# fal-ai-community/video-diffusion-speedrun

Hardware: AMD Instinct MI355X
Metric: train-step samples/sec (video latents) (higher is better)
Workload: dtype bf16; 1 GPU; C3b DiT-XL/2 bf16, latents [16,16,64,64] pt=2 -> 8192+16 tokens, ctx [512,4096]; per_gpu_batch=12, global_batch=12, parallelism=single, launch=eager, deterministic=False

## Files before the change

### video_diffusion_speedrun_amd/csrc/gemm.hip

```cpp
#include "common.h"
#include "prof.h"
#include "config.h"
#include "../../include/vds.h"
#include <cmath>
#include <cstdint>
#include <cstring>
#include <mutex>
#include <type_traits>

#ifndef VDS_GEMM_AUX_NT
#define VDS_GEMM_AUX_NT 1
#endif
namespace {

constexpr int BM = 128, BN = 128, BK = 64;
constexpr int TILE_BYTES = 16384;
constexpr int EPI_LD = 68;
constexpr int LDS_BYTES = 4 * 64 * EPI_LD * 4;
constexpr int GROUP_M = 8;

struct GemmP {
  int M, N, K;
  const bf16_t* A; long lda;
  const bf16_t* B; long ldb;
// ... 233 lines not shown
      const float g[8] = {g0[0], g0[1], g0[2], g0[3], g1[0], g1[1], g1[2], g1[3]};
      const u32x4 xr = auxr[it];
      u32x4 o, o2;
#pragma unroll
      for (int e = 0; e < 4; ++e) {
        float a = v[2 * e] + bias8[2 * e], bb = v[2 * e + 1] + bias8[2 * e + 1];
        o[e] = pack_bf2(a, bb);
        o2[e] = pack_bf2(bflo(xr[e]) + a * g[2 * e], bfhi(xr[e]) + bb * g[2 * e + 1]);
      }
      if (p.C) *reinterpret_cast<u32x4*>(reinterpret_cast<bf16_t*>(p.C) + grow * p.ldc + gcol) = o;
      *reinterpret_cast<u32x4*>(reinterpret_cast<bf16_t*>(p.C2) + grow * p.ldc2 + gcol) = o2;
    } else if constexpr (EPI == VDS_EPI_DGELU) {
      const u32x4 pr = auxr[it];
      u32x4 o;
#pragma unroll
      for (int e = 0; e < 4; ++e) {
        if constexpr (LUT) o[e] = f2_to_bf2(f32x2{v[2 * e], v[2 * e + 1]} * lut_pair(lut, pr[e]));
        else o[e] = pack_bf2(v[2 * e] * dgelu_f(bflo(pr[e])), v[2 * e + 1] * dgelu_f(bfhi(pr[e])));
      }
      if (p.C) *reinterpret_cast<u32x4*>(reinterpret_cast<bf16_t*>(p.C) + grow * p.ldc + gcol) = o;
      if constexpr (EMIT) ev = o;
    }
    if constexpr (EMIT) {
      float f[8];
#pragma unroll
      for (int e = 0; e < 4; ++e) { f[2 * e] = bflo(ev[e]); f[2 * e + 1] = bfhi(ev[e]); }
      if (p.e_colsum)
#pragma unroll
        for (int e = 0; e < 8; ++e) cs[e] += f[e];
      if (emit) {
#pragma unroll
        for (int e = 0; e < 8; ++e) {
          e_max = fmaxf(e_max, fabsf(f[e]));
          f[e] = fminf(fmaxf(f[e] * e_scale, -e_fmax), e_fmax);
        }
        const u32x2 w = {cvt4_fp8(p.e_fmt, f[0], f[1], f[2], f[3]), cvt4_fp8(p.e_fmt, f[4], f[5], f[6], f[7])};
        ew[it] = w;
        if (p.e_q) *reinterpret_cast<u32x2*>(p.e_q + grow * p.e_ldq + gcol) = w;
      }
    }
  }
  if constexpr (EMIT) {
    if (emit) {
      if (p.e_amax_out) {
#pragma unroll
        for (int o = 32; o > 0; o >>= 1) e_max = fmaxf(e_max, __shfl_xor(e_max, o));
        unsigned* a = reinterpret_cast<unsigned*>(p.e_amax_out);
        if (lane == 0 && __float_as_uint(e_max) > __atomic_load_n(a, __ATOMIC_RELAXED)) atomicMax(a, __float_as_uint(e_max));
      }
    }
  }
}

template <int EPI, int EFMT, bool C1, bool C2, bool EQ, bool CS, int WC = 64, int NIT = 8>
__device__ __forceinline__ void epilogue_full(const GemmP& p, const float* stg, const char* lut, int row0, int col0, int lane,
                                              float (&cs)[8], u32x2 (&ew)[NIT], const u32x4 (&auxr)[NIT], float e_scale,
                                              float& e_max) {
  const int c8 = lane & 7, rin = lane >> 3;
  if constexpr (WC < 64) {
    if (c8 * 8 >= WC) {
      if constexpr (EQ) {
#pragma unroll
        for (int it = 0; it < NIT; ++it) ew[it] = u32x2{0u, 0u};
      }
      return;
    }
  }
  const int gcol = col0 + c8 * 8;
  const long grow0 = row0 + rin;
  f32x2 bias[4];
#pragma unroll
  for (int e = 0; e < 4; ++e) bias[e] = f32x2{0.f, 0.f};
  if constexpr (EPI == VDS_EPI_STORE || EPI == VDS_EPI_BIAS_GELU || EPI == VDS_EPI_GATE_RES) {
    if (p.bias) {
      const u32x4 bv = *reinterpret_cast<const u32x4*>(p.bias + gcol);
#pragma unroll
      for (int e = 0; e < 4; ++e) bias[e] = bf2_to_f2(bv[e]);
    }
  }
  [[maybe_unused]] f32x2 g[4];
  if constexpr (EPI == VDS_EPI_GATE_RES) {
    const float* gp = p.gate + (long)((row0 + p.row_base) / p.rows_per_batch) * p.ldgate + gcol;
    const f32x4 g0 = *reinterpret_cast<const f32x4*>(gp), g1 = *reinterpret_cast<const f32x4*>(gp + 4);
    g[0] = f32x2{g0[0], g0[1]}; g[1] = f32x2{g0[2], g0[3]}; g[2] = f32x2{g1[0], g1[1]}; g[3] = f32x2{g1[2], g1[3]};
  }
  [[maybe_unused]] bf16_t* c1 = reinterpret_cast<bf16_t*>(p.C) + grow0 * p.ldc + gcol;
  [[maybe_unused]] bf16_t* c2 = reinterpret_cast<bf16_t*>(p.C2) + grow0 * p.ldc2 + gcol;
  [[maybe_unused]] unsigned char* eq = p.e_q + grow0 * p.e_ldq + gcol;
  const long s1 = 8 * p.ldc, s2 = 8 * p.ldc2, sq = 8 * p.e_ldq;
  constexpr float FMAX = EFMT == 0 ? 448.0f : 57344.0f;
  const float* sp = stg + rin * EPI_LD + c8 * 8;
#pragma unroll
  for (int it = 0; it < NIT; ++it) {
    const f32x4 lo = *reinterpret_cast<const f32x4*>(sp + it * 8 * EPI_LD);
    const f32x4 hi = *reinterpret_cast<const f32x4*>(sp + it * 8 * EPI_LD + 4);
    const f32x2 v[4] = {f32x2{lo[0], lo[1]}, f32x2{lo[2], lo[3]}, f32x2{hi[0], hi[1]}, f32x2{hi[2], hi[3]}};
    [[maybe_unused]] u32x4 ev;
    if constexpr (EPI == VDS_EPI_STORE) {
      u32x4 o;
#pragma unroll
      for (int e = 0; e < 4; ++e) o[e] = f2_to_bf2(v[e] + bias[e]);
      __builtin_nontemporal_store(o, reinterpret_cast<u32x4*>(c1 + it * s1));
    } else if constexpr (EPI == VDS_EPI_BIAS_GELU) {
      u32x4 o, o2;
#pragma unroll
      for (int e = 0; e < 4; ++e) {
        o[e] = f2_to_bf2(v[e] + bias[e]);
        o2[e] = f2_to_bf2(bf2_to_f2(o[e]) * lut_pair(lut, o[e]));
      }
      if constexpr (C1) __builtin_nontemporal_store(o, reinterpret_cast<u32x4*>(c1 + it * s1));
      if constexpr (C2) __builtin_nontemporal_store(o2, reinterpret_cast<u32x4*>(c2 + it * s2));
      ev = o2;
    } else if constexpr (EPI == VDS_EPI_GATE_RES) {
      const u32x4 xr = auxr[it];
      u32x4 o, o2;
#pragma unroll
      for (int e = 0; e < 4; ++e) {
        const f32x2 a = v[e] + bias[e];
        o[e] = f2_to_bf2(a);
        o2[e] = f2_to_bf2(bf2_to_f2(xr[e]) + a * g[e]);
      }
      if constexpr (C1) __builtin_nontemporal_store(o, reinterpret_cast<u32x4*>(c1 + it * s1));
      __builtin_nontemporal_store(o2, reinterpret_cast<u32x4*>(c2 + it * s2));
    } else if constexpr (EPI == VDS_EPI_DGELU) {
      const u32x4 pr = auxr[it];
      u32x4 o;
#pragma unroll
      for (int e = 0; e < 4; ++e) o[e] = f2_to_bf2(v[e] * lut_pair(lut, pr[e]));
      if constexpr (C1) __builtin_nontemporal_store(o, reinterpret_cast<u32x4*>(c1 + it * s1));
      ev = o;
    }
    if constexpr (EQ || CS) {
      f32x2 f[4];
#pragma unroll
      for (int e = 0; e < 4; ++e) f[e] = bf2_to_f2(ev[e]);
      if constexpr (CS)
#pragma unroll
        for (int e = 0; e < 4; ++e) { cs[2 * e] += f[e][0]; cs[2 * e + 1] += f[e][1]; }
      if constexpr (EQ) {
        float q[8];
#pragma unroll
        for (int e = 0; e < 4; ++e) {
          e_max = fmaxf(fmaxf(e_max, fabsf(f[e][0])), fabsf(f[e][1]));
          const f32x2 sc = f[e] * e_scale;
          q[2 * e] = __builtin_amdgcn_fmed3f(sc[0], -FMAX, FMAX);
          q[2 * e + 1] = __builtin_amdgcn_fmed3f(sc[1], -FMAX, FMAX);
        }
        const u32x2 w = {fp8_cvt4<EFMT>(q[0], q[1], q[2], q[3]), fp8_cvt4<EFMT>(q[4], q[5], q[6], q[7])};
        ew[it] = w;
        *reinterpret_cast<u32x2*>(eq + it * sq) = w;
      }
    }
  }
}

template <int EPI, bool EMIT, int WC = 64, int NIT = 8>
__device__ __forceinline__ bool epilogue_full_dispatch(const GemmP& p, const float* stg, const char* lut, int row0, int col0,
                                                       int lane, float (&cs)[8], u32x2 (&ew)[NIT], const u32x4 (&auxr)[NIT],
                                                       float e_scale, float& e_max) {
  const bool c1 = p.C != nullptr, c2 = p.C2 != nullptr;
  [[maybe_unused]] bool eq = false, eany = false, csum = false;
  if constexpr (EMIT) {
    eq = p.e_q != nullptr;
    eany = p.e_q || p.e_qt;
    csum = p.e_colsum != nullptr;
  }
#define VDS_FULL(E, F, A, B, Q, S) epilogue_full<E, F, A, B, Q, S, WC, NIT>(p, stg, lut, row0, col0, lane, cs, ew, auxr, e_scale, e_max)
  if constexpr (EPI == VDS_EPI_STORE) {
    VDS_FULL(EPI, 0, true, false, false, false);
    return true;
  } else if constexpr (EPI == VDS_EPI_GATE_RES) {
    if (c1) VDS_FULL(EPI, 0, true, true, false, false);
    else VDS_FULL(EPI, 0, false, true, false, false);
    return true;
  } else if constexpr (EPI == VDS_EPI_BIAS_GELU) {
    if (c1 && c2 && !eany) { VDS_FULL(EPI, 0, true, true, false, false); return true; }
    if (!c1 && c2 && !eany) { VDS_FULL(EPI, 0, false, true, false, false); return true; }
    if constexpr (EMIT) {
      if (c1 && !c2 && eq && !csum && p.e_fmt == 0) { VDS_FULL(EPI, 0, true, false, true, false); return true; }
    }
    return false;
  } else if constexpr (EPI == VDS_EPI_DGELU) {
    if (c1 && !eany && !csum) { VDS_FULL(EPI, 0, true, false, false, false); return true; }
    if constexpr (EMIT) {
      if (c1 && !eany && csum) { VDS_FULL(EPI, 0, true, false, false, true); return true; }
      if (!c1 && eq && csum && p.e_fmt == 1) { VDS_FULL(EPI, 1, false, false, true, true); return true; }
      if (!c1 && eq && !csum && p.e_fmt == 1) { VDS_FULL(EPI, 1, false, false, true, false); return true; }
    }
    return false;
  } else {
    return false;
  }
#undef VDS_FULL
}

template <int LAYOUT, int EPI>
__global__ __launch_bounds__(256, 2) void gemm_kernel(GemmP p) {
  extern __shared__ __attribute__((aligned(16))) char smem[];
  constexpr bool A_KM = (LAYOUT == VDS_TN);
  constexpr bool B_KM = (LAYOUT != VDS_NT);
  const int tid = threadIdx.x, lane = tid & 63;
  const int wave = __builtin_amdgcn_readfirstlane(tid >> 6);
  const int wm = wave >> 1, wn = wave & 1;

  const int nwg = p.tiles_m * p.tiles_n;
  int pid = blockIdx.x;
  {
    int q = nwg >> 3, r = nwg & 7, xcd = pid & 7, idx = pid >> 3;
    pid = (xcd < r ? xcd * (q + 1) : r * (q + 1) + (xcd - r) * q) + idx;
  }
  const int group = GROUP_M * p.tiles_n;
  const int first_m = (pid / group) * GROUP_M;
  const int gsz = min(p.tiles_m - first_m, GROUP_M);
  const int tile_m = first_m + (pid % group) % gsz;
  const int tile_n = (pid % group) / gsz;
  const int m0 = tile_m * BM, n0 = tile_n * BN;

  const int kt_total = (p.K + BK - 1) / BK;
  int kt_begin = 0, kt_end = kt_total;
  if (p.split_k > 1) {
    int per = (kt_total + p.split_k - 1) / p.split_k;
    kt_begin = blockIdx.y * per;
    kt_end = min(kt_total, kt_begin + per);
    if (kt_begin >= kt_end) return;
  }

  const srd_t ra = make_srd(p.A, p.a_bytes);
  const srd_t rb = make_srd(p.B, p.b_bytes);
  unsigned va[4], vb[4];
  stage_offsets<A_KM>(va, wave, lane, p.lda, m0);
  stage_offsets<B_KM>(vb, wave, lane, p.ldb, n0);
  const unsigned a_step = A_KM ? (unsigned)(BK * p.lda * 2) : BK * 2;
  const unsigned b_step = B_KM ? (unsigned)(BK * p.ldb * 2) : BK * 2;


  f32x4 acc[4][4];
#pragma unroll
  for (int i = 0; i < 4; ++i)
#pragma unroll
    for (int j = 0; j < 4; ++j) acc[i][j] = f32x4{0.f, 0.f, 0.f, 0.f};

  stage_tile<A_KM>(ra, smem, va, kt_begin * a_step, wave, lane, p.K - kt_begin * BK);
  stage_tile<B_KM>(rb, smem + TILE_BYTES, vb, kt_begin * b_step, wave, lane, p.K - kt_begin * BK);
  VDS_WAIT_VM(0);
// ... 64 lines not shown

template <int G, int STRIDE, int OFF>
__device__ __forceinline__ int to_tile(int local) { return (local / G) * STRIDE + OFF + (local % G); }

__device__ __forceinline__ int swz8(int row) { return ((row >> 1) & 3) | ((row >> 3) & 4); }
__device__ __forceinline__ i32x8 frag_km8(const char* tile, int db, int lane) {
  const int m = lane & 15, g = lane >> 4, q = m >> 1, pp = m & 1;
  const int st = ((q >> 1) & 3) | ((g & 1) << 2);
  const char* p = tile + (32 * g + q) * 128 + ((db ^ st) << 4) + 8 * pp;
  i32x8 r;
#pragma unroll
  for (int t = 0; t < 4; ++t) {
    typedef __attribute__((ext_vector_type(2))) int i32x2_t;
    const i32x2_t w = __builtin_amdgcn_ds_read_tr8_b64_v2i32((__attribute__((address_space(3))) i32x2_t*)LDS_PTR(p + t * 8 * 128));
    r[2 * t] = w[0];
    r[2 * t + 1] = w[1];
  }
  return r;
}
template <int G, int STRIDE, int OFF>
__device__ __forceinline__ void half_offsets_km8(unsigned (&voff)[2], int (&kchunk)[2], int wave, int lane, long ld_bytes,
                                                 int origin) {
#pragma unroll
  for (int j = 0; j < 2; ++j) {
    const int row = (wave * 2 + j) * 8 + (lane >> 3);
    const int chunk = (lane & 7) ^ swz8(row);
    kchunk[j] = 0;
    voff[j] = (unsigned)((long)row * ld_bytes + origin + to_tile<G, STRIDE, OFF>(chunk * 16));
  }
}

template <bool KMAJOR, int G, int STRIDE, int OFF, int NP>
__device__ __forceinline__ void half_offsets(unsigned (&voff)[NP], int (&kchunk)[NP], int wave, int lane, long ld,
                                             int origin) {
#pragma unroll
  for (int j = 0; j < NP; ++j) {
    const int q = wave * NP + j;
    if constexpr (!KMAJOR) {
      const int row = q * 8 + (lane >> 3);
      const int chunk = swz_kc(row, lane & 7);
      kchunk[j] = chunk * 8;
      voff[j] = (unsigned)(((long)(origin + to_tile<G, STRIDE, OFF>(row)) * ld + chunk * 8) * 2);
    } else {
      static_assert(NP == 2, "half-tiles are staged as two 1-KiB pieces per wave");
      const int krow = q * 4 + (lane >> 4);
      const int pc = lane & 15;
      const int chunk = (((pc >> 1) ^ swz_km(krow)) << 1) | (pc & 1);
      kchunk[j] = 0;
      voff[j] = (unsigned)(((long)krow * ld + origin + to_tile<G, STRIDE, OFF>(chunk * 8)) * 2);
    }
  }
}

template <bool KMAJOR, int NP = 2>
__device__ __forceinline__ void issue_half(srd_t rsrc, char* slot, const unsigned (&voff)[NP],
                                           const int (&kchunk)[NP], unsigned koff, int krem, int wave) {
  const unsigned base = lds_addr_of(slot) + wave * (NP * 1024);
#pragma unroll
  for (int j = 0; j < NP; ++j) {
    unsigned off = voff[j] + koff;
    if constexpr (!KMAJOR) {
      if (kchunk[j] >= krem) off = 0xfffffff0u;
    } else {
      if (krem <= 0) off = 0xfffffff0u;
    }
    lds_dma16(rsrc, base + j * 1024, off);
  }
}

template <int LAYOUT, int EPI, int FMT, int WN>
__device__ __forceinline__ void gemm_tile(const GemmP& p, char* smem, const int m0, const int n0, const int kt_begin,
                                          const int kt_end) {
  static_assert(FMT == 0 || (FMT != 3 && LAYOUT == VDS_NT) || (FMT == 3 && LAYOUT == VDS_TN),
                "fp8 operands: k-contiguous (FMT 1 / 2, NT) or both k-major (FMT 3, TN: the weight gradient)");
  using G = Geo<WN>;
  constexpr int WCOLS = G::WCOLS, NJ = G::NJ, BUF = G::BUF;
  constexpr int SLOT_A0 = G::A0, SLOT_A1 = G::A1, SLOT_B0 = G::B0, SLOT_B1 = G::B1;
  constexpr int NPB1 = 2;
  constexpr bool A_KM = (LAYOUT == VDS_TN);
  constexpr bool B_KM = (LAYOUT != VDS_NT);
  const int tid = threadIdx.x, lane = tid & 63;
  const int wave = __builtin_amdgcn_readfirstlane(tid >> 6);
  const int wr = wave >> 2, wc = wave & 3;
  const srd_t ra = make_srd(p.A, p.a_bytes);
  const srd_t rb = make_srd(p.B, p.b_bytes);
  constexpr bool USE_LUT = EPI == VDS_EPI_BIAS_GELU || EPI == VDS_EPI_DGELU;
  char* const ring = smem + (USE_LUT ? LUT_BYTES : 0);
  if (USE_LUT) {
    const srd_t rl = make_srd(g_gelu_lut[EPI == VDS_EPI_DGELU ? 1 : 0], LUT_BYTES);
    const unsigned lb = lds_addr_of(smem) + wave * 2048;
    lds_dma16(rl, lb, (unsigned)(wave * 2048 + lane * 16));
    lds_dma16(rl, lb + 1024, (unsigned)(wave * 2048 + 1024 + lane * 16));
  }
  unsigned va[2][2], vb0[2], vb1[NPB1];
  int ca[2][2], cb0[2], cb1[NPB1];
  if constexpr (FMT == 3) {
    half_offsets_km8<64, 128, 0>(va[0], ca[0], wave, lane, 2 * p.lda, m0);
    half_offsets_km8<64, 128, 64>(va[1], ca[1], wave, lane, 2 * p.lda, m0);
    if constexpr (WN == 128) {
      half_offsets_km8<32, 32, 0>(vb0, cb0, wave, lane, 2 * p.ldb, n0);
    } else {
      half_offsets_km8<32, 64, 0>(vb0, cb0, wave, lane, 2 * p.ldb, n0);
      half_offsets_km8<32, 64, 32>(vb1, cb1, wave, lane, 2 * p.ldb, n0);
    }
  } else {
  half_offsets<A_KM, 64, 128, 0, 2>(va[0], ca[0], wave, lane, p.lda, m0);
  half_offsets<A_KM, 64, 128, 64, 2>(va[1], ca[1], wave, lane, p.lda, m0);
  }
  if constexpr (FMT == 3) {
  } else if constexpr (WN == 128) {
    half_offsets<B_KM, 32, 32, 0, 2>(vb0, cb0, wave, lane, p.ldb, n0);
  } else {
    half_offsets<B_KM, 32, 64, 0, 2>(vb0, cb0, wave, lane, p.ldb, n0);
    half_offsets<B_KM, 32, 64, 32, 2>(vb1, cb1, wave, lane, p.ldb, n0);
  }
  const unsigned a_step = A_KM ? (unsigned)((FMT == 3 ? 2 * BK : BK) * p.lda * 2) : BK * 2;
  const unsigned b_step = B_KM ? (unsigned)((FMT == 3 ? 2 * BK : BK) * p.ldb * 2) : BK * 2;

  auto issue = [&](int T, int which, int par) {
    const int krem = (T < kt_end) ? p.K - T * BK : 0;
    char* buf = ring + par * BUF;
    if (which == 0) issue_half<A_KM>(ra, buf + SLOT_A0, va[0], ca[0], (unsigned)T * a_step, krem, wave);
    else if (which == 3) issue_half<A_KM>(ra, buf + SLOT_A1, va[1], ca[1], (unsigned)T * a_step, krem, wave);
    else if (which == 1) issue_half<B_KM>(rb, buf + SLOT_B0, vb0, cb0, (unsigned)T * b_step, krem, wave);
    else if constexpr (WN != 128) issue_half<B_KM, NPB1>(rb, buf + SLOT_B1, vb1, cb1, (unsigned)T * b_step, krem, wave);
  };

  f32x4 acc[8][NJ];
#pragma unroll
  for (int i = 0; i < 8; ++i)
#pragma unroll
    for (int j = 0; j < NJ; ++j) {
      acc[i][j] = f32x4{0.f, 0.f, 0.f, 0.f};
      if constexpr (LAYOUT != VDS_TN) asm volatile("" : "+v"(acc[i][j]));
    }

  constexpr int KS = FMT == 0 ? 2 : 1;
  using frag_t = std::conditional_t<FMT == 0, bf16x8, i32x8>;
  auto mma = [&](const frag_t& a, const frag_t& b, f32x4 c) {
    if constexpr (FMT == 0) return __builtin_amdgcn_mfma_f32_16x16x32_bf16(b, a, c, 0, 0, 0);
    else return __builtin_amdgcn_mfma_scale_f32_16x16x128_f8f6f4(b, a, c, 0, FMT >= 2 ? 1 : 0, 0, 0, 0, 0);
  };
  auto read_a4 = [&](const char* slot, frag_t (&fa)[4][KS]) {
#pragma unroll
    for (int i = 0; i < 4; ++i)
#pragma unroll
      for (int ks = 0; ks < KS; ++ks) {
        if constexpr (FMT == 3) fa[i][ks] = frag_km8(slot, wr * 4 + i, lane);
        else if constexpr (FMT != 0) fa[i][ks] = frag_kc8(slot, wr * 64 + i * 16, lane);
        else if constexpr (A_KM) fa[i][ks] = frag_km(slot, wr * 64 + i * 16, ks, lane);
        else fa[i][ks] = frag_kc(slot, wr * 64 + i * 16, ks, lane);
      }
  };
  auto read_b2 = [&](const char* slot, frag_t (&fb)[2][KS]) {
#pragma unroll
    for (int j = 0; j < 2; ++j)
#pragma unroll
      for (int ks = 0; ks < KS; ++ks) {
        if constexpr (FMT == 3) fb[j][ks] = frag_km8(slot, wc * 2 + j, lane);
        else if constexpr (FMT != 0) fb[j][ks] = frag_kc8(slot, wc * 32 + j * 16, lane);
        else if constexpr (B_KM) fb[j][ks] = frag_km(slot, wc * 32 + j * 16, ks, lane);
        else fb[j][ks] = frag_kc(slot, wc * 32 + j * 16, ks, lane);
      }
  };

  if constexpr (WN == 256) {
  issue(kt_begin, 0, 0); issue(kt_begin, 1, 0); issue(kt_begin, 2, 0); issue(kt_begin, 3, 0);
  issue(kt_begin + 1, 0, 1); issue(kt_begin + 1, 1, 1); issue(kt_begin + 1, 2, 1);
  VDS_WAIT_VM(8);
  __builtin_amdgcn_s_barrier();
  if (wr == 1) __builtin_amdgcn_s_barrier();
  frag_t fa[4][KS], fb0[2][KS], fb1[2][KS];
  auto quad = [&](int qa, int qb, frag_t (&fb)[2][KS]) {
#pragma unroll
    for (int ks = 0; ks < KS; ++ks)
#pragma unroll
      for (int i = 0; i < 4; ++i)
#pragma unroll
        for (int j = 0; j < 2; ++j) acc[qa * 4 + i][qb * 2 + j] = mma(fa[i][ks], fb[j][ks], acc[qa * 4 + i][qb * 2 + j]);
  };
  auto k_tile = [&](int T, auto PAR) {
    constexpr int par = decltype(PAR)::value;
    const char* buf = ring + par * BUF;
    read_a4(buf + SLOT_A0, fa);
    read_b2(buf + SLOT_B0, fb0);
    read_b2(buf + SLOT_B1, fb1);
    issue(T + 1, 3, par ^ 1);
    VDS_WAIT_LGKM0();
    VDS_WAIT_VM(8);
    __builtin_amdgcn_s_barrier();
    __builtin_amdgcn_s_setprio(1);
    quad(0, 0, fb0);
    quad(0, 1, fb1);
    __builtin_amdgcn_s_setprio(0);
    __builtin_amdgcn_s_barrier();
    read_a4(buf + SLOT_A1, fa);
    issue(T + 2, 0, par);
    issue(T + 2, 1, par);
    issue(T + 2, 2, par);
    VDS_WAIT_LGKM0();
    VDS_WAIT_VM(8);
    __builtin_amdgcn_s_barrier();
    __builtin_amdgcn_s_setprio(1);
    quad(1, 1, fb1);
    quad(1, 0, fb0);
    __builtin_amdgcn_s_setprio(0);
    __builtin_amdgcn_s_barrier();
  };
  for (int T = kt_begin; T < kt_end; T += 2) {
    k_tile(T, std::integral_constant<int, 0>{});
    if (T + 1 < kt_end) k_tile(T + 1, std::integral_constant<int, 1>{});
  }
  } else {
  static_assert(WN == 128, "tile widths: 256, and 128 for a narrow last tile column");
  issue(kt_begin, 0, 0); issue(kt_begin, 1, 0); issue(kt_begin, 3, 0);
  issue(kt_begin + 1, 0, 1); issue(kt_begin + 1, 1, 1);
  VDS_WAIT_VM(6);
  __builtin_amdgcn_s_barrier();
  if (wr == 1) __builtin_amdgcn_s_barrier();
  frag_t fa[4][KS], fb0[2][KS];
  auto quad = [&](int qa) {
#pragma unroll
    for (int ks = 0; ks < KS; ++ks)
#pragma unroll
      for (int i = 0; i < 4; ++i)
#pragma unroll
        for (int j = 0; j < 2; ++j) acc[qa * 4 + i][j] = mma(fa[i][ks], fb0[j][ks], acc[qa * 4 + i][j]);
  };
  auto k_tile = [&](int T, auto PAR) {
    constexpr int par = decltype(PAR)::value;
    const char* buf = ring + par * BUF;
    read_a4(buf + SLOT_A0, fa);
    read_b2(buf + SLOT_B0, fb0);
    issue(T + 1, 3, par ^ 1);
    VDS_WAIT_LGKM0();
    VDS_WAIT_VM(6);
    __builtin_amdgcn_s_barrier();
    __builtin_amdgcn_s_setprio(1);
    quad(0);
    __builtin_amdgcn_s_setprio(0);
    __builtin_amdgcn_s_barrier();
    read_a4(buf + SLOT_A1, fa);
    issue(T + 2, 0, par);
    issue(T + 2, 1, par);
    VDS_WAIT_LGKM0();
    VDS_WAIT_VM(6);
    __builtin_amdgcn_s_barrier();
    __builtin_amdgcn_s_setprio(1);
    quad(1);
    __builtin_amdgcn_s_setprio(0);
    __builtin_amdgcn_s_barrier();
  };
  for (int T = kt_begin; T < kt_end; T += 2) {
    k_tile(T, std::integral_constant<int, 0>{});
    if (T + 1 < kt_end) k_tile(T + 1, std::integral_constant<int, 1>{});
  }
  }
  constexpr int NIT = 8;
  constexpr int NSTEP = 16 / NIT;
  constexpr int RSTEP = 8 * NIT;
  u32x4 auxr2[NSTEP][NIT];
#pragma unroll
  for (int st = 0; st < NSTEP; ++st)
    epilogue_prefetch<EPI, G::WCOLS, NIT>(p, m0 + wr * 128 + st * RSTEP, n0 + wc * G::WCOLS, lane, auxr2[st]);
  if (wr == 0) __builtin_amdgcn_s_barrier();
  const bool aux_all = (EPI == VDS_EPI_GATE_RES || EPI == VDS_EPI_DGELU) && m0 + wr * 128 + 128 <= p.M &&
                       n0 + (wc + 1) * G::WCOLS <= p.N;
  if (aux_all) VDS_WAIT_VM(16);
  else VDS_WAIT_VM(0);
  __builtin_amdgcn_s_barrier();

  constexpr int STG_BASE = 0, STG_WAVE = RSTEP * EPI_LD;
  float* stg = reinterpret_cast<float*>(ring + STG_BASE) + wave * STG_WAVE;
  float dq = 1.0f;
  if constexpr (FMT != 0) dq = (p.sa ? *p.sa : 1.0f) * (p.sb ? *p.sb : 1.0f);
  constexpr bool EMIT = (FMT != 0 && (EPI == VDS_EPI_BIAS_GELU || EPI == VDS_EPI_DGELU)) || (FMT == 0 && EPI == VDS_EPI_DGELU);
  float cs[8];
  u32x2 ew[NSTEP][NIT];
#pragma unroll
  for (int e = 0; e < 8; ++e) cs[e] = 0.f;
  [[maybe_unused]] float e_scale = 1.0f, e_max = 0.f;
  if constexpr (EMIT) {
    const float fmax = p.e_fmt == 0 ? 448.0f : 57344.0f;
    const float ain = ((p.e_q || p.e_qt) && p.e_amax_in) ? *p.e_amax_in : 0.f;
    e_scale = ain > 0.f ? fmax / ain : 1.0f;
    if ((p.e_q || p.e_qt) && p.e_dq_out && m0 == 0 && n0 == 0 && tid == 0) *p.e_dq_out = ain > 0.f ? ain / fmax : 1.0f;
  }
  const char* lut = smem;
#pragma unroll
  for (int qa = 0; qa < NSTEP; ++qa) {
    const u32x4 (&auxr)[NIT] = auxr2[qa];
    const int row0 = m0 + wr * 128 + qa * RSTEP, col0 = n0 + wc * WCOLS;
#pragma unroll
    for (int i = 0; i < RSTEP / 16; ++i)
#pragma unroll
      for (int j = 0; j < NJ; ++j) {
        f32x4 v = acc[qa * (RSTEP / 16) + i][j];
        if constexpr (FMT != 0) v *= dq;
        *reinterpret_cast<f32x4*>(stg + (i * 16 + (lane & 15)) * EPI_LD + j * 16 + 4 * (lane >> 4)) = v;
      }
    VDS_WAIT_LGKM0();
    __builtin_amdgcn_wave_barrier();
    bool full = row0 + RSTEP <= p.M && col0 + WCOLS <= p.N;
    if constexpr (EPI == VDS_EPI_GATE_RES) full = full && ((row0 + p.row_base) % p.rows_per_batch) + RSTEP <= p.rows_per_batch;
    if constexpr (EPI == VDS_EPI_F32) full = false;
    bool done = false;
    if (full) done = epilogue_full_dispatch<EPI, EMIT, WCOLS, NIT>(p, stg, lut, row0, col0, lane, cs, ew[qa], auxr, e_scale, e_max);
    if (!done) epilogue_64x64<EPI, EMIT, USE_LUT, WCOLS, NIT>(p, stg, row0, col0, lane, cs, ew[qa], auxr, lut);
    __builtin_amdgcn_wave_barrier();
  }
  if constexpr (EMIT) {
    if ((p.e_q || p.e_qt) && p.e_amax_out) {
#pragma unroll
      for (int o = 32; o > 0; o >>= 1) e_max = fmaxf(e_max, __shfl_xor(e_max, o));
      unsigned* a = reinterpret_cast<unsigned*>(p.e_amax_out);
      if (lane == 0 && __float_as_uint(e_max) > __atomic_load_n(a, __ATOMIC_RELAXED)) atomicMax(a, __float_as_uint(e_max));
    }
  }
  if constexpr (EMIT) {
    if (p.e_qt) {
      constexpr int TLD = 72;
      unsigned char* bt = reinterpret_cast<unsigned char*>(stg);
      const int c8 = lane & 7, rin = lane >> 3;
#pragma unroll
      for (int qa = 0; qa < NSTEP; ++qa)
#pragma unroll
        for (int it = 0; it < NIT; ++it) *reinterpret_cast<u32x2*>(bt + (qa * RSTEP + it * 8 + rin) * TLD + c8 * 8) = ew[qa][it];
      VDS_WAIT_LGKM0();
      __builtin_amdgcn_wave_barrier();
      const int mq = lane & 31;
      const long m = m0 + wr * 128 + 4 * mq;
#pragma unroll
      for (int it = 0; it < 8; ++it) {
        const int kq = (lane >> 5) + 2 * it;
        unsigned r[4];
#pragma unroll
        for (int i = 0; i < 4; ++i) r[i] = *reinterpret_cast<const unsigned*>(bt + (4 * mq + i) * TLD + 4 * kq);
        const unsigned t0 = __builtin_amdgcn_perm(r[1], r[0], 0x05010400u), t1 = __builtin_amdgcn_perm(r[1], r[0], 0x07030602u);
        const unsigned t2 = __builtin_amdgcn_perm(r[3], r[2], 0x05010400u), t3 = __builtin_amdgcn_perm(r[3], r[2], 0x07030602u);
        const unsigned c[4] = {__builtin_amdgcn_perm(t2, t0, 0x05040100u), __builtin_amdgcn_perm(t2, t0, 0x07060302u),
                               __builtin_amdgcn_perm(t3, t1, 0x05040100u), __builtin_amdgcn_perm(t3, t1, 0x07060302u)};
#pragma unroll
        for (int j = 0; j < 4; ++j) {
          const int col = n0 + wc * WCOLS + 4 * kq + j;
          if (col >= p.N || m >= p.M || 4 * kq + j >= WCOLS) continue;
          unsigned char* dst = p.e_qt + (long)col * p.e_ldqt + m;
          if (m + 4 <= p.M) *reinterpret_cast<unsigned*>(dst) = c[j];
          else
            for (int i = 0; i < (int)(p.M - m); ++i) dst[i] = (unsigned char)(c[j] >> (8 * i));
        }
      }
      VDS_WAIT_LGKM0();
      __builtin_amdgcn_wave_barrier();
    }
    if (p.e_colsum) {
#pragma unroll
      for (int e = 0; e < 8; ++e) {
        cs[e] += __shfl_xor(cs[e], 8);
        cs[e] += __shfl_xor(cs[e], 16);
        cs[e] += __shfl_xor(cs[e], 32);
      }
      if (wr == 1 && lane < 8)
#pragma unroll
        for (int e = 0; e < 8; ++e) stg[lane * 8 + e] = cs[e];
      __syncthreads();
      if (wr == 0 && lane < WCOLS / 8) {
        const float* other = reinterpret_cast<const float*>(ring + STG_BASE) + (wave + 4) * STG_WAVE;
        const int gcol = n0 + wc * WCOLS + lane * 8;
#pragma unroll
        for (int e = 0; e < 8; ++e)
          if (gcol + e < p.N) atomicAdd(p.e_colsum + gcol + e, cs[e] + other[lane * 8 + e]);
      }
    }
  }
}

template <int LAYOUT, int EPI, int FMT = 0>
__global__ __launch_bounds__(512, 2) void gemm_kernel(GemmP p) {
  extern __shared__ __attribute__((aligned(16))) char smem[];
  const int nwg = p.tiles_m * p.tiles_n;
  int pid = blockIdx.x;
  {
    int q = nwg >> 3, r = nwg & 7, xcd = pid & 7, idx = pid >> 3;
    pid = (xcd < r ? xcd * (q + 1) : r * (q + 1) + (xcd - r) * q) + idx;
  }
  const int group = p.group_m * p.tiles_n;
  const int first_m = (pid / group) * p.group_m;
  const int gsz = min(p.tiles_m - first_m, p.group_m);
  const int tile_m = first_m + (pid % group) % gsz;
  const int tile_n = (pid % group) / gsz;
  const int m0 = tile_m * BM, n0 = tile_n * 256;

  const int kt_total = (p.K + BK - 1) / BK;
  int kt_begin = 0, kt_end = kt_total;
  if (p.split_k > 1) {
    int per = (kt_total + p.split_k - 1) / p.split_k;
    kt_begin = blockIdx.y * per;
    kt_end = min(kt_total, kt_begin + per);
    if (kt_begin >= kt_end) return;
  }
  if (p.narrow && tile_n == p.tiles_n - 1) {
    gemm_tile<LAYOUT, EPI, FMT, 128>(p, smem, m0, n0, kt_begin, kt_end);
    return;
  }
  gemm_tile<LAYOUT, EPI, FMT, 256>(p, smem, m0, n0, kt_begin, kt_end);
}

template <int LAYOUT, int EPI, int FMT = 0>
int launch(const GemmP& p, hipStream_t s) {
  constexpr bool USE_LUT = EPI == VDS_EPI_BIAS_GELU || EPI == VDS_EPI_DGELU;
  constexpr int LDS_TOTAL = LDS_BYTES + (USE_LUT ? LUT_BYTES : 0);
  static bool attr_set = false;
  if (!attr_set) {
    (void)hipFuncSetAttribute(reinterpret_cast<const void*>(&gemm_kernel<LAYOUT, EPI, FMT>),
                              hipFuncAttributeMaxDynamicSharedMemorySize, LDS_TOTAL);
    attr_set = true;
  }
  if constexpr (USE_LUT) {
    if (!ensure_gelu_lut()) return VDS_ERR_LAUNCH;
  }
  dim3 grid(p.tiles_m * p.tiles_n, p.split_k > 1 ? p.split_k : 1, 1);
  const double k = FMT != 0 ? p.prof_k : (double)p.K;
  vdsprof::Scope ps(FMT != 0 ? VDS_PROF_GEMM_FP8 : LAYOUT == VDS_NT ? VDS_PROF_GEMM_NT : LAYOUT == VDS_NN ? VDS_PROF_GEMM_NN
                                                                                                       : VDS_PROF_GEMM_TN,
                    s, 2.0 * p.M * p.N * k, (FMT != 0 ? 1.0 : 2.0) * ((double)p.M * k + (double)p.N * k) + 2.0 * (double)p.M * p.N);
  hipLaunchKernelGGL((gemm_kernel<LAYOUT, EPI, FMT>), grid, dim3(512), LDS_TOTAL, s, p);
  return hipGetLastError() == hipSuccess ? VDS_OK : VDS_ERR_LAUNCH;
}

}

namespace mid {
constexpr int BM = 256, BN = 128, BK = 32;
constexpr int A_BYTES = 16384, B_BYTES = 8192, STAGE = A_BYTES + B_BYTES;
constexpr int LDS_BYTES = 3 * STAGE;
static_assert(LDS_BYTES >= 4 * 64 * EPI_LD * 4, "epilogue staging must fit in the stage ring");

__device__ __forceinline__ int swz32(int row) {
  const int h = (row >> 2) & 3;
  return (((h >> 1) ^ h) & 1) << 1 | (h >> 1);
}

template <bool KMAJOR, int ROWS>
__device__ __forceinline__ void offsets(unsigned (&voff)[ROWS / 64], int (&kchunk)[ROWS / 64], int wave, int lane,
                                        long ld, int origin) {
  constexpr int NP = ROWS / 64;
#pragma unroll
  for (int j = 0; j < NP; ++j) {
    const int q = wave * NP + j;
    if constexpr (!KMAJOR) {
      const int row = q * 16 + (lane >> 2);
      const int chunk = (lane & 3) ^ swz32(row);
      kchunk[j] = chunk * 8;
      voff[j] = (unsigned)(((long)(origin + row) * ld + chunk * 8) * 2);
    } else {
      const int t = q >> 3, krow = (q & 7) * 4 + (lane >> 4);
      const int pc = lane & 15;
      const int chunk = (((pc >> 1) ^ swz_km(krow)) << 1) | (pc & 1);
      kchunk[j] = krow;
      voff[j] = (unsigned)(((long)krow * ld + origin + t * 128 + chunk * 8) * 2);
    }
  }
}

template <bool KMAJOR, int NP>
__device__ __forceinline__ void issue(srd_t rsrc, char* slot, const unsigned (&voff)[NP], const int (&kchunk)[NP],
                                      unsigned koff, int krem, int wave) {
  const unsigned base = lds_addr_of(slot) + wave * NP * 1024;
#pragma unroll
  for (int j = 0; j < NP; ++j) {
    unsigned off = voff[j] + koff;
    if (kchunk[j] >= krem) off = 0xfffffff0u;
    lds_dma16(rsrc, base + j * 1024, off);
  }
// ... 446 lines not shown
```

Before: 14.80 samples/s.

## Make NT/NN GEMM persistent with next-tile prologue overlapped into epilogue

Converts the NT and NN GEMM kernels into a persistent tile loop launched with one workgroup per CU. Each workgroup issues the first K-tile loads of its next output tile during the current tile's epilogue, and tracks outstanding vmcnt so the pipeline carries across tiles. Bias and gate vectors are prefetched before the epilogue. The aim is to hide prologue and epilogue latency and cut launch/tail costs. The trade-offs are fewer concurrent workgroups (one per CU instead of up to two resident), a smaller epilogue chunk, and split-K being rejected for these layouts.

```diff
diff --git a/video_diffusion_speedrun_amd/csrc/gemm.hip b/video_diffusion_speedrun_amd/csrc/gemm.hip
--- a/video_diffusion_speedrun_amd/csrc/gemm.hip
+++ b/video_diffusion_speedrun_amd/csrc/gemm.hip
@@ -309,10 +309,11 @@
   }
 }
 
+struct EpiPre { u32x4 bias; f32x4 g0, g1; };
 template <int EPI, int EFMT, bool C1, bool C2, bool EQ, bool CS, int WC = 64, int NIT = 8>
 __device__ __forceinline__ void epilogue_full(const GemmP& p, const float* stg, const char* lut, int row0, int col0, int lane,
                                               float (&cs)[8], u32x2 (&ew)[NIT], const u32x4 (&auxr)[NIT], float e_scale,
-                                              float& e_max) {
+                                              float& e_max, bool use_pre = false, const EpiPre& pre = EpiPre{}) {
   const int c8 = lane & 7, rin = lane >> 3;
   if constexpr (WC < 64) {
     if (c8 * 8 >= WC) {
@@ -329,7 +330,10 @@
 #pragma unroll
   for (int e = 0; e < 4; ++e) bias[e] = f32x2{0.f, 0.f};
   if constexpr (EPI == VDS_EPI_STORE || EPI == VDS_EPI_BIAS_GELU || EPI == VDS_EPI_GATE_RES) {
-    if (p.bias) {
+    if (use_pre) {
+#pragma unroll
+      for (int e = 0; e < 4; ++e) bias[e] = bf2_to_f2(pre.bias[e]);
+    } else if (p.bias) {
       const u32x4 bv = *reinterpret_cast<const u32x4*>(p.bias + gcol);
 #pragma unroll
       for (int e = 0; e < 4; ++e) bias[e] = bf2_to_f2(bv[e]);
@@ -337,8 +341,13 @@
   }
   [[maybe_unused]] f32x2 g[4];
   if constexpr (EPI == VDS_EPI_GATE_RES) {
-    const float* gp = p.gate + (long)((row0 + p.row_base) / p.rows_per_batch) * p.ldgate + gcol;
-    const f32x4 g0 = *reinterpret_cast<const f32x4*>(gp), g1 = *reinterpret_cast<const f32x4*>(gp + 4);
+    f32x4 g0, g1;
+    if (use_pre) {
+      g0 = pre.g0; g1 = pre.g1;
+    } else {
+      const float* gp = p.gate + (long)((row0 + p.row_base) / p.rows_per_batch) * p.ldgate + gcol;
+      g0 = *reinterpret_cast<const f32x4*>(gp); g1 = *reinterpret_cast<const f32x4*>(gp + 4);
+    }
     g[0] = f32x2{g0[0], g0[1]}; g[1] = f32x2{g0[2], g0[3]}; g[2] = f32x2{g1[0], g1[1]}; g[3] = f32x2{g1[2], g1[3]};
   }
   [[maybe_unused]] bf16_t* c1 = reinterpret_cast<bf16_t*>(p.C) + grow0 * p.ldc + gcol;
@@ -412,9 +421,9 @@
 }
 
 template <int EPI, bool EMIT, int WC = 64, int NIT = 8>
-__device__ __forceinline__ bool epilogue_full_dispatch(const GemmP& p, const float* stg, const char* lut, int row0, int col0,
+__device__ __forceinline__ int epilogue_full_dispatch(const GemmP& p, const float* stg, const char* lut, int row0, int col0,
                                                        int lane, float (&cs)[8], u32x2 (&ew)[NIT], const u32x4 (&auxr)[NIT],
-                                                       float e_scale, float& e_max) {
+                                                       float e_scale, float& e_max, bool use_pre = false, const EpiPre& pre = EpiPre{}) {
   const bool c1 = p.C != nullptr, c2 = p.C2 != nullptr;
   [[maybe_unused]] bool eq = false, eany = false, csum = false;
   if constexpr (EMIT) {
@@ -422,31 +431,31 @@
     eany = p.e_q || p.e_qt;
     csum = p.e_colsum != nullptr;
   }
-#define VDS_FULL(E, F, A, B, Q, S) epilogue_full<E, F, A, B, Q, S, WC, NIT>(p, stg, lut, row0, col0, lane, cs, ew, auxr, e_scale, e_max)
+#define VDS_FULL(E, F, A, B, Q, S) epilogue_full<E, F, A, B, Q, S, WC, NIT>(p, stg, lut, row0, col0, lane, cs, ew, auxr, e_scale, e_max, use_pre, pre)
   if constexpr (EPI == VDS_EPI_STORE) {
     VDS_FULL(EPI, 0, true, false, false, false);
-    return true;
+    return 1;
   } else if constexpr (EPI == VDS_EPI_GATE_RES) {
     if (c1) VDS_FULL(EPI, 0, true, true, false, false);
     else VDS_FULL(EPI, 0, false, true, false, false);
-    return true;
+    return c1 ? 2 : 1;
   } else if constexpr (EPI == VDS_EPI_BIAS_GELU) {
-    if (c1 && c2 && !eany) { VDS_FULL(EPI, 0, true, true, false, false); return true; }
-    if (!c1 && c2 && !eany) { VDS_FULL(EPI, 0, false, true, false, false); return true; }
+    if (c1 && c2 && !eany) { VDS_FULL(EPI, 0, true, true, false, false); return 2; }
+    if (!c1 && c2 && !eany) { VDS_FULL(EPI, 0, false, true, false, false); return 1; }
     if constexpr (EMIT) {
-      if (c1 && !c2 && eq && !csum && p.e_fmt == 0) { VDS_FULL(EPI, 0, true, false, true, false); return true; }
-    }
-    return false;
+      if (c1 && !c2 && eq && !csum && p.e_fmt == 0) { VDS_FULL(EPI, 0, true, false, true, false); return 2; }
+    }
+    return 0;
   } else if constexpr (EPI == VDS_EPI_DGELU) {
-    if (c1 && !eany && !csum) { VDS_FULL(EPI, 0, true, false, false, false); return true; }
+    if (c1 && !eany && !csum) { VDS_FULL(EPI, 0, true, false, false, false); return 1; }
     if constexpr (EMIT) {
-      if (c1 && !eany && csum) { VDS_FULL(EPI, 0, true, false, false, true); return true; }
-      if (!c1 && eq && csum && p.e_fmt == 1) { VDS_FULL(EPI, 1, false, false, true, true); return true; }
-      if (!c1 && eq && !csum && p.e_fmt == 1) { VDS_FULL(EPI, 1, false, false, true, false); return true; }
-    }
-    return false;
+      if (c1 && !eany && csum) { VDS_FULL(EPI, 0, true, false, false, true); return 1; }
+      if (!c1 && eq && csum && p.e_fmt == 1) { VDS_FULL(EPI, 1, false, false, true, true); return 1; }
+      if (!c1 && eq && !csum && p.e_fmt == 1) { VDS_FULL(EPI, 1, false, false, true, false); return 1; }
+    }
+    return 0;
   } else {
-    return false;
+    return 0;
   }
 #undef VDS_FULL
 }
@@ -617,6 +626,15 @@
   }
 }
 
+__device__ __forceinline__ void lds_dma16_ws(srd_t srd, unsigned lds, unsigned voff) {
+  unsigned keep;
+  asm volatile(
+      "s_mov_b32 %0, m0\n\ts_mov_b32 m0, %1\n\ts_nop 2\n\tbuffer_load_dwordx4 %2, %3, 0 offen lds\n\ts_mov_b32 m0, %0"
+      : "=&s"(keep)
+      : "s"(lds), "v"(voff), "s"(srd)
+      : "memory");
+}
+
 template <bool KMAJOR, int NP = 2>
 __device__ __forceinline__ void issue_half(srd_t rsrc, char* slot, const unsigned (&voff)[NP],
                                            const int (&kchunk)[NP], unsigned koff, int krem, int wave) {
@@ -629,13 +647,51 @@
     } else {
       if (krem <= 0) off = 0xfffffff0u;
     }
-    lds_dma16(rsrc, base + j * 1024, off);
-  }
-}
-
-template <int LAYOUT, int EPI, int FMT, int WN>
-__device__ __forceinline__ void gemm_tile(const GemmP& p, char* smem, const int m0, const int n0, const int kt_begin,
-                                          const int kt_end) {
+    lds_dma16_ws(rsrc, base + j * 1024, off);
+  }
+}
+
+template <int BASE>
+__device__ __forceinline__ void wait_vm_plus(int s) {
+  static_assert(BASE + 32 <= 63, "vmcnt is a 6-bit counter");
+  if (s >= 32) asm volatile("s_waitcnt vmcnt(%0)" ::"n"(BASE + 32) : "memory");
+  else if (s >= 16) asm volatile("s_waitcnt vmcnt(%0)" ::"n"(BASE + 16) : "memory");
+  else asm volatile("s_waitcnt vmcnt(%0)" ::"n"(BASE) : "memory");
+}
+
+template <int LAYOUT, int WNX>
+__device__ __forceinline__ void issue_first_k_tile(const GemmP& p, char* ring, int m0, int n0, int kt_begin, int wave, int lane) {
+  using G = Geo<WNX>;
+  constexpr bool A_KM = (LAYOUT == VDS_TN);
+  constexpr bool B_KM = (LAYOUT != VDS_NT);
+  const srd_t ra = make_srd(p.A, p.a_bytes);
+  const srd_t rb = make_srd(p.B, p.b_bytes);
+  const unsigned a_step = A_KM ? (unsigned)(BK * p.lda * 2) : BK * 2;
+  const unsigned b_step = B_KM ? (unsigned)(BK * p.ldb * 2) : BK * 2;
+  const int krem = p.K - kt_begin * BK;
+  unsigned v[2];
+  int c[2];
+  half_offsets<A_KM, 64, 128, 0, 2>(v, c, wave, lane, p.lda, m0);
+  issue_half<A_KM>(ra, ring + G::A0, v, c, (unsigned)kt_begin * a_step, krem, wave);
+  if constexpr (WNX == 128) {
+    half_offsets<B_KM, 32, 32, 0, 2>(v, c, wave, lane, p.ldb, n0);
+    issue_half<B_KM>(rb, ring + G::B0, v, c, (unsigned)kt_begin * b_step, krem, wave);
+  } else {
+    half_offsets<B_KM, 32, 64, 0, 2>(v, c, wave, lane, p.ldb, n0);
+    issue_half<B_KM>(rb, ring + G::B0, v, c, (unsigned)kt_begin * b_step, krem, wave);
+    half_offsets<B_KM, 32, 64, 32, 2>(v, c, wave, lane, p.ldb, n0);
+    issue_half<B_KM>(rb, ring + G::B1, v, c, (unsigned)kt_begin * b_step, krem, wave);
+  }
+  half_offsets<A_KM, 64, 128, 64, 2>(v, c, wave, lane, p.lda, m0);
+  issue_half<A_KM>(ra, ring + G::A1, v, c, (unsigned)kt_begin * a_step, krem, wave);
+}
+
+template <int LAYOUT, int EPI, int FMT, int WN, bool PERSIST = false>
+__device__ __forceinline__ int gemm_tile(const GemmP& p, char* smem, const int m0, const int n0, const int kt_begin,
+                                         const int kt_end, [[maybe_unused]] const bool first = true,
+                                         [[maybe_unused]] const int carry = 0, [[maybe_unused]] const int next_kind = 0,
+                                         [[maybe_unused]] const int next_m0 = 0, [[maybe_unused]] const int next_n0 = 0) {
+  static_assert(!PERSIST || (LAYOUT != VDS_TN && FMT != 3 && EPI != VDS_EPI_F32), "tile loop: NT / NN, no split-K");
   static_assert(FMT == 0 || (FMT != 3 && LAYOUT == VDS_NT) || (FMT == 3 && LAYOUT == VDS_TN),
                 "fp8 operands: k-contiguous (FMT 1 / 2, NT) or both k-major (FMT 3, TN: the weight gradient)");
   using G = Geo<WN>;
@@ -644,18 +700,20 @@
   constexpr int NPB1 = 2;
   constexpr bool A_KM = (LAYOUT == VDS_TN);
   constexpr bool B_KM = (LAYOUT != VDS_NT);
-  const int tid = threadIdx.x, lane = tid & 63;
+  int tid = threadIdx.x;
+  if constexpr (PERSIST) asm volatile("" : "+v"(tid));
+  int lane = tid & 63;
   const int wave = __builtin_amdgcn_readfirstlane(tid >> 6);
   const int wr = wave >> 2, wc = wave & 3;
   const srd_t ra = make_srd(p.A, p.a_bytes);
   const srd_t rb = make_srd(p.B, p.b_bytes);
   constexpr bool USE_LUT = EPI == VDS_EPI_BIAS_GELU || EPI == VDS_EPI_DGELU;
   char* const ring = smem + (USE_LUT ? LUT_BYTES : 0);
-  if (USE_LUT) {
+  if (USE_LUT && first) {
     const srd_t rl = make_srd(g_gelu_lut[EPI == VDS_EPI_DGELU ? 1 : 0], LUT_BYTES);
     const unsigned lb = lds_addr_of(smem) + wave * 2048;
-    lds_dma16(rl, lb, (unsigned)(wave * 2048 + lane * 16));
-    lds_dma16(rl, lb + 1024, (unsigned)(wave * 2048 + 1024 + lane * 16));
+    lds_dma16_ws(rl, lb, (unsigned)(wave * 2048 + lane * 16));
+    lds_dma16_ws(rl, lb + 1024, (unsigned)(wave * 2048 + 1024 + lane * 16));
   }
   unsigned va[2][2], vb0[2], vb1[NPB1];
   int ca[2][2], cb0[2], cb1[NPB1];
@@ -730,10 +788,17 @@
   };
 
   if constexpr (WN == 256) {
-  issue(kt_begin, 0, 0); issue(kt_begin, 1, 0); issue(kt_begin, 2, 0); issue(kt_begin, 3, 0);
-  issue(kt_begin + 1, 0, 1); issue(kt_begin + 1, 1, 1); issue(kt_begin + 1, 2, 1);
-  VDS_WAIT_VM(8);
-  __builtin_amdgcn_s_barrier();
+  if (!PERSIST || first) {
+    issue(kt_begin, 0, 0); issue(kt_begin, 1, 0); issue(kt_begin, 2, 0); issue(kt_begin, 3, 0);
+    issue(kt_begin + 1, 0, 1); issue(kt_begin + 1, 1, 1); issue(kt_begin + 1, 2, 1);
+    VDS_WAIT_VM(8);
+    __builtin_amdgcn_s_barrier();
+  } else {
+    VDS_WAIT_LGKM0();
+    wait_vm_plus<2>(carry);
+    __builtin_amdgcn_s_barrier();
+    issue(kt_begin + 1, 0, 1); issue(kt_begin + 1, 1, 1); issue(kt_begin + 1, 2, 1);
+  }
   if (wr == 1) __builtin_amdgcn_s_barrier();
   frag_t fa[4][KS], fb0[2][KS], fb1[2][KS];
   auto quad = [&](int qa, int qb, frag_t (&fb)[2][KS]) {
@@ -744,7 +809,7 @@
 #pragma unroll
         for (int j = 0; j < 2; ++j) acc[qa * 4 + i][qb * 2 + j] = mma(fa[i][ks], fb[j][ks], acc[qa * 4 + i][qb * 2 + j]);
   };
-  auto k_tile = [&](int T, auto PAR) {
+  auto k_tile = [&](int T, auto PAR, auto HEAD) {
     constexpr int par = decltype(PAR)::value;
     const char* buf = ring + par * BUF;
     read_a4(buf + SLOT_A0, fa);
@@ -752,7 +817,8 @@
     read_b2(buf + SLOT_B1, fb1);
     issue(T + 1, 3, par ^ 1);
     VDS_WAIT_LGKM0();
-    VDS_WAIT_VM(8);
+    if constexpr (decltype(HEAD)::value) wait_vm_plus<8>(carry);
+    else VDS_WAIT_VM(8);
     __builtin_amdgcn_s_barrier();
     __builtin_amdgcn_s_setprio(1);
     quad(0, 0, fb0);
@@ -772,16 +838,29 @@
     __builtin_amdgcn_s_setprio(0);
     __builtin_amdgcn_s_barrier();
   };
-  for (int T = kt_begin; T < kt_end; T += 2) {
-    k_tile(T, std::integral_constant<int, 0>{});
-    if (T + 1 < kt_end) k_tile(T + 1, std::integral_constant<int, 1>{});
+  int T0 = kt_begin;
+  if constexpr (PERSIST) {
+    k_tile(T0, std::integral_constant<int, 0>{}, std::true_type{});
+    if (T0 + 1 < kt_end) k_tile(T0 + 1, std::integral_constant<int, 1>{}, std::false_type{});
+    T0 += 2;
+  }
+  for (int T = T0; T < kt_end; T += 2) {
+    k_tile(T, std::integral_constant<int, 0>{}, std::false_type{});
+    if (T + 1 < kt_end) k_tile(T + 1, std::integral_constant<int, 1>{}, std::false_type{});
   }
   } else {
   static_assert(WN == 128, "tile widths: 256, and 128 for a narrow last tile column");
-  issue(kt_begin, 0, 0); issue(kt_begin, 1, 0); issue(kt_begin, 3, 0);
-  issue(kt_begin + 1, 0, 1); issue(kt_begin + 1, 1, 1);
-  VDS_WAIT_VM(6);
-  __builtin_amdgcn_s_barrier();
+  if (!PERSIST || first) {
+    issue(kt_begin, 0, 0); issue(kt_begin, 1, 0); issue(kt_begin, 3, 0);
+    issue(kt_begin + 1, 0, 1); issue(kt_begin + 1, 1, 1);
+    VDS_WAIT_VM(6);
+    __builtin_amdgcn_s_barrier();
+  } else {
+    VDS_WAIT_LGKM0();
+    wait_vm_plus<2>(carry);
+    __builtin_amdgcn_s_barrier();
+    issue(kt_begin + 1, 0, 1); issue(kt_begin + 1, 1, 1);
+  }
   if (wr == 1) __builtin_amdgcn_s_barrier();
   frag_t fa[4][KS], fb0[2][KS];
   auto quad = [&](int qa) {
@@ -792,14 +871,15 @@
 #pragma unroll
         for (int j = 0; j < 2; ++j) acc[qa * 4 + i][j] = mma(fa[i][ks], fb0[j][ks], acc[qa * 4 + i][j]);
   };
-  auto k_tile = [&](int T, auto PAR) {
+  auto k_tile = [&](int T, auto PAR, auto HEAD) {
     constexpr int par = decltype(PAR)::value;
     const char* buf = ring + par * BUF;
     read_a4(buf + SLOT_A0, fa);
     read_b2(buf + SLOT_B0, fb0);
     issue(T + 1, 3, par ^ 1);
     VDS_WAIT_LGKM0();
-    VDS_WAIT_VM(6);
+    if constexpr (decltype(HEAD)::value) wait_vm_plus<6>(carry);
+    else VDS_WAIT_VM(6);
     __builtin_amdgcn_s_barrier();
     __builtin_amdgcn_s_setprio(1);
     quad(0);
@@ -816,26 +896,71 @@
     __builtin_amdgcn_s_setprio(0);
     __builtin_amdgcn_s_barrier();
   };
-  for (int T = kt_begin; T < kt_end; T += 2) {
-    k_tile(T, std::integral_constant<int, 0>{});
-    if (T + 1 < kt_end) k_tile(T + 1, std::integral_constant<int, 1>{});
-  }
-  }
-  constexpr int NIT = 8;
+  int T0 = kt_begin;
+  if constexpr (PERSIST) {
+    k_tile(T0, std::integral_constant<int, 0>{}, std::true_type{});
+    if (T0 + 1 < kt_end) k_tile(T0 + 1, std::integral_constant<int, 1>{}, std::false_type{});
+    T0 += 2;
+  }
+  for (int T = T0; T < kt_end; T += 2) {
+    k_tile(T, std::integral_constant<int, 0>{}, std::false_type{});
+    if (T + 1 < kt_end) k_tile(T + 1, std::integral_constant<int, 1>{}, std::false_type{});
+  }
+  }
+  constexpr int NIT = PERSIST ? 4 : 8;
   constexpr int NSTEP = 16 / NIT;
   constexpr int RSTEP = 8 * NIT;
   u32x4 auxr2[NSTEP][NIT];
+  if constexpr (PERSIST) asm volatile("" : "+v"(lane));
 #pragma unroll
   for (int st = 0; st < NSTEP; ++st)
     epilogue_prefetch<EPI, G::WCOLS, NIT>(p, m0 + wr * 128 + st * RSTEP, n0 + wc * G::WCOLS, lane, auxr2[st]);
+  [[maybe_unused]] EpiPre pre_v;
+  [[maybe_unused]] bool use_pre = false;
+  if constexpr (PERSIST) {
+    const int prow = m0 + wr * 128, pcol = n0 + wc * G::WCOLS + (lane & 7) * 8;
+    pre_v.bias = u32x4{0u, 0u, 0u, 0u};
+    pre_v.g0 = pre_v.g1 = f32x4{0.f, 0.f, 0.f, 0.f};
+    bool ok = prow + 128 <= p.M && n0 + (wc + 1) * G::WCOLS <= p.N;
+    if constexpr (EPI == VDS_EPI_GATE_RES)
+      ok = ok && (prow + p.row_base) / p.rows_per_batch == (prow + 127 + p.row_base) / p.rows_per_batch;
+    if (ok) {
+      const bool cok = pcol + 8 <= p.N;
+      if constexpr (EPI != VDS_EPI_DGELU) {
+        if (p.bias && cok) pre_v.bias = *reinterpret_cast<const u32x4*>(p.bias + pcol);
+      }
+      if constexpr (EPI == VDS_EPI_GATE_RES) {
+        if (cok) {
+          const float* gp = p.gate + (long)((prow + p.row_base) / p.rows_per_batch) * p.ldgate + pcol;
+          pre_v.g0 = *reinterpret_cast<const f32x4*>(gp);
+          pre_v.g1 = *reinterpret_cast<const f32x4*>(gp + 4);
+        }
+      }
+      use_pre = true;
+    }
+  }
   if (wr == 0) __builtin_amdgcn_s_barrier();
-  const bool aux_all = (EPI == VDS_EPI_GATE_RES || EPI == VDS_EPI_DGELU) && m0 + wr * 128 + 128 <= p.M &&
+  const bool aux_all = !PERSIST && (EPI == VDS_EPI_GATE_RES || EPI == VDS_EPI_DGELU) && m0 + wr * 128 + 128 <= p.M &&
                        n0 + (wc + 1) * G::WCOLS <= p.N;
   if (aux_all) VDS_WAIT_VM(16);
   else VDS_WAIT_VM(0);
   __builtin_amdgcn_s_barrier();
-
-  constexpr int STG_BASE = 0, STG_WAVE = RSTEP * EPI_LD;
+  if constexpr (PERSIST) {
+    if constexpr (EPI == VDS_EPI_GATE_RES || EPI == VDS_EPI_DGELU) {
+#pragma unroll
+      for (int st = 0; st < NSTEP; ++st)
+#pragma unroll
+        for (int it = 0; it < NIT; ++it) asm volatile("" ::"v"(auxr2[st][it]));
+    }
+    asm volatile("" ::"v"(pre_v.bias), "v"(pre_v.g0), "v"(pre_v.g1));
+    if (next_kind == 1) issue_first_k_tile<LAYOUT, 256>(p, ring, next_m0, next_n0, kt_begin, wave, lane);
+    else if (next_kind == 2) issue_first_k_tile<LAYOUT, 128>(p, ring, next_m0, next_n0, kt_begin, wave, lane);
+  }
+
+  constexpr int STG_BASE = PERSIST ? BUF : 0;
+  constexpr int STG_WAVE = PERSIST ? 9216 / 4 : RSTEP * EPI_LD;
+  static_assert(STG_WAVE >= RSTEP * EPI_LD && STG_BASE + 8 * STG_WAVE * 4 <= LDS_BYTES, "staging area");
+  [[maybe_unused]] int n_stores = 0;
   float* stg = reinterpret_cast<float*>(ring + STG_BASE) + wave * STG_WAVE;
   float dq = 1.0f;
   if constexpr (FMT != 0) dq = (p.sa ? *p.sa : 1.0f) * (p.sb ? *p.sb : 1.0f);
@@ -869,8 +994,9 @@
     bool full = row0 + RSTEP <= p.M && col0 + WCOLS <= p.N;
     if constexpr (EPI == VDS_EPI_GATE_RES) full = full && ((row0 + p.row_base) % p.rows_per_batch) + RSTEP <= p.rows_per_batch;
     if constexpr (EPI == VDS_EPI_F32) full = false;
-    bool done = false;
-    if (full) done = epilogue_full_dispatch<EPI, EMIT, WCOLS, NIT>(p, stg, lut, row0, col0, lane, cs, ew[qa], auxr, e_scale, e_max);
+    int done = 0;
+    if (full) done = epilogue_full_dispatch<EPI, EMIT, WCOLS, NIT>(p, stg, lut, row0, col0, lane, cs, ew[qa], auxr, e_scale, e_max, use_pre, pre_v);
+    n_stores += done * NIT;
     if (!done) epilogue_64x64<EPI, EMIT, USE_LUT, WCOLS, NIT>(p, stg, row0, col0, lane, cs, ew[qa], auxr, lut);
     __builtin_amdgcn_wave_barrier();
   }
@@ -928,7 +1054,12 @@
       if (wr == 1 && lane < 8)
 #pragma unroll
         for (int e = 0; e < 8; ++e) stg[lane * 8 + e] = cs[e];
-      __syncthreads();
+      if constexpr (PERSIST) {
+        VDS_WAIT_LGKM0();
+        __builtin_amdgcn_s_barrier();
+      } else {
+        __syncthreads();
+      }
       if (wr == 0 && lane < WCOLS / 8) {
         const float* other = reinterpret_cast<const float*>(ring + STG_BASE) + (wave + 4) * STG_WAVE;
         const int gcol = n0 + wc * WCOLS + lane * 8;
@@ -938,13 +1069,13 @@
       }
     }
   }
-}
-
-template <int LAYOUT, int EPI, int FMT = 0>
-__global__ __launch_bounds__(512, 2) void gemm_kernel(GemmP p) {
-  extern __shared__ __attribute__((aligned(16))) char smem[];
+  if constexpr (PERSIST) return __builtin_amdgcn_readfirstlane(n_stores);
+  else return 0;
+}
+
+__device__ __forceinline__ void tile_of(const GemmP& p, int id, int& m0, int& n0, int& narrow) {
   const int nwg = p.tiles_m * p.tiles_n;
-  int pid = blockIdx.x;
+  int pid = id;
   {
     int q = nwg >> 3, r = nwg & 7, xcd = pid & 7, idx = pid >> 3;
     pid = (xcd < r ? xcd * (q + 1) : r * (q + 1) + (xcd - r) * q) + idx;
@@ -954,7 +1085,39 @@
   const int gsz = min(p.tiles_m - first_m, p.group_m);
   const int tile_m = first_m + (pid % group) % gsz;
   const int tile_n = (pid % group) / gsz;
-  const int m0 = tile_m * BM, n0 = tile_n * 256;
+  m0 = tile_m * BM;
+  n0 = tile_n * 256;
+  narrow = p.narrow && tile_n == p.tiles_n - 1;
+}
+
+template <int LAYOUT, int EPI>
+constexpr bool kTileLoop = LAYOUT != VDS_TN && EPI != VDS_EPI_F32;
+
+template <int LAYOUT, int EPI, int FMT = 0>
+__global__ __launch_bounds__(512, 2) void gemm_kernel(GemmP p) {
+  extern __shared__ __attribute__((aligned(16))) char smem[];
+  if constexpr (kTileLoop<LAYOUT, EPI>) {
+    const int nwg = p.tiles_m * p.tiles_n, G = gridDim.x;
+    const int kt_end = (p.K + BK - 1) / BK;
+    int id = blockIdx.x, m0, n0, narrow, carry = 0;
+    bool first = true;
+    tile_of(p, id, m0, n0, narrow);
+    for (;;) {
+      int next_kind = 0, nm0 = 0, nn0 = 0, nnarrow = 0;
+      if (id + G < nwg) {
+        tile_of(p, id + G, nm0, nn0, nnarrow);
+        next_kind = nnarrow ? 2 : 1;
+      }
+      if (narrow) carry = gemm_tile<LAYOUT, EPI, FMT, 128, true>(p, smem, m0, n0, 0, kt_end, first, carry, next_kind, nm0, nn0);
+      else carry = gemm_tile<LAYOUT, EPI, FMT, 256, true>(p, smem, m0, n0, 0, kt_end, first, carry, next_kind, nm0, nn0);
+      if (!next_kind) break;
+      id += G; m0 = nm0; n0 = nn0; narrow = nnarrow;
+      first = false;
+    }
+    VDS_WAIT_VM(0);
+  } else {
+  int m0, n0, narrow;
+  tile_of(p, blockIdx.x, m0, n0, narrow);
 
   const int kt_total = (p.K + BK - 1) / BK;
   int kt_begin = 0, kt_end = kt_total;
@@ -964,11 +1127,24 @@
     kt_end = min(kt_total, kt_begin + per);
     if (kt_begin >= kt_end) return;
   }
-  if (p.narrow && tile_n == p.tiles_n - 1) {
+  if (narrow) {
     gemm_tile<LAYOUT, EPI, FMT, 128>(p, smem, m0, n0, kt_begin, kt_end);
     return;
   }
   gemm_tile<LAYOUT, EPI, FMT, 256>(p, smem, m0, n0, kt_begin, kt_end);
+  }
+}
+
+inline int cu_count() {
+  static int cached[64] = {};
+  int dev = 0;
+  if (hipGetDevice(&dev) != hipSuccess || dev < 0 || dev >= 64) return 0;
+  if (!cached[dev]) {
+    int n = 0;
+    if (hipDeviceGetAttribute(&n, hipDeviceAttributeMultiprocessorCount, dev) != hipSuccess || n < 8) return 0;
+    cached[dev] = n & ~7;
+  }
+  return cached[dev];
 }
 
 template <int LAYOUT, int EPI, int FMT = 0>
@@ -984,7 +1160,14 @@
   if constexpr (USE_LUT) {
     if (!ensure_gelu_lut()) return VDS_ERR_LAUNCH;
   }
-  dim3 grid(p.tiles_m * p.tiles_n, p.split_k > 1 ? p.split_k : 1, 1);
+  int tiles = p.tiles_m * p.tiles_n;
+  if constexpr (kTileLoop<LAYOUT, EPI>) {
+    if (p.split_k > 1) return VDS_ERR_ARG;
+    const int cus = cu_count();
+    if (cus <= 0) return VDS_ERR_LAUNCH;
+    if (tiles > cus) tiles = cus;
+  }
+  dim3 grid(tiles, p.split_k > 1 ? p.split_k : 1, 1);
   const double k = FMT != 0 ? p.prof_k : (double)p.K;
   vdsprof::Scope ps(FMT != 0 ? VDS_PROF_GEMM_FP8 : LAYOUT == VDS_NT ? VDS_PROF_GEMM_NT : LAYOUT == VDS_NN ? VDS_PROF_GEMM_NN
                                                                                                        : VDS_PROF_GEMM_TN,
```

Measured after the change: 14.69 samples/s. About the same (-0.7%).
